# fancifulland2718/mujoco_InverseDynamicsTest

Measured on AMD Instinct MI355X. Metric: mj_inverse evals/sec, humanoid 27-DoF, batch=65536 @ 1/2/4/8 MI355X vs host CPU, higher is better.
Workload: dtype f64; 1 GPU; humanoid 27-DoF mj_inverse (skipstage NONE), contacts disabled, nefc=0, full mjData mirror written; per_gpu_batch=65536, global_batch=65536, parallelism=dp1

## Files before the change

include/mjhip.h:

```cpp
#ifndef MJHIP_H_
#define MJHIP_H_

#include <stddef.h>
#include <stdint.h>

#include "mjhip_fields.h"

#ifdef __cplusplus
extern "C" {
#endif

#if defined(_WIN32)
  #define MJHIP_API __declspec(dllexport)
#else
  #define MJHIP_API __attribute__((visibility("default")))
#endif

typedef double mjtNum;
typedef unsigned char mjtByte;

#define mjhipPI      3.14159265358979323846
#define mjhipMINVAL  1E-15
#define mjhipMAXVAL  1E+10
#define mjhipMINIMP  0.0001
// ... 197 lines not shown
MJHIP_API int mjhip_contextCreate(const mjhipModel* m, int device, int capacity,
                                  mjhipContext** out);
MJHIP_API int mjhip_contextCreateCapped(const mjhipModel* m, int device, int capacity,
                                        int max_contacts, int max_rows, mjhipContext** out);
MJHIP_API void mjhip_contextFree(mjhipContext* c);
MJHIP_API int mjhip_contextCapacity(const mjhipContext* c);
MJHIP_API const char* mjhip_contextFastKernel(const mjhipContext* c);
MJHIP_API int mjhip_contextFastKernelLds(const mjhipContext* c);
MJHIP_API int mjhip_contextLoadKernel(mjhipContext* c, const void* image, size_t size,
                                      const char* name, unsigned long long signature,
                                      int cmode);
MJHIP_API int mjhip_contextLastPath(const mjhipContext* c);
MJHIP_API int mjhip_contextConstStores(const mjhipContext* c);
MJHIP_API int mjhip_contextConstLaunches(const mjhipContext* c);
MJHIP_API int mjhip_contextQmHandoff(const mjhipContext* c);
MJHIP_API const char* mjhip_contextConstraintKernel(const mjhipContext* c);
MJHIP_API int mjhip_worklistCount(mjhipContext* c);
MJHIP_API void* mjhip_contextStream(mjhipContext* c);
MJHIP_API int mjhip_contextSetStream(mjhipContext* c, void* stream);

MJHIP_API int mjhip_inverseBatch(mjhipContext* c, int B,
                                 const mjtNum* qpos, const mjtNum* qvel, const mjtNum* qacc,
                                 mjtNum* qfrc_inverse, int skipstage, int skipsensor,
                                 int flags, int* status);

MJHIP_API int mjhip_forwardBatch(mjhipContext* c, int B, const mjtNum* qpos, const mjtNum* qvel,
                                 const mjtNum* ctrl, mjtNum* qacc, int flags, int* status);

MJHIP_API int mjhip_forwardBatchEx(mjhipContext* c, int B, const mjtNum* qpos,
                                   const mjtNum* qvel, const mjtNum* ctrl, const mjtNum* act,
// ... 134 lines not shown
```

mujoco_inversedynamicstest_amd/codegen.py:

```python
from __future__ import annotations

import hashlib
import re

import numpy as np

from . import fields

FREE, BALL, SLIDE, HINGE = 0, 1, 2, 3
STAGES = ("pos", "fac", "va")
FRAMES_IN_PASS1 = True
MAX_LDS_HINGES = 32
PREFETCH = 1
FUSE = True
VA_RECOMPUTE = False
QM_HANDOFF = True
QM_ORDER = "late"
QM_HANDOFF_MIN_B = 49152
VA_LDS_SLOTS = None
VA_KEEP_QFP = True
LDS_BUDGET = 40960
LANES = {"pos": 64, "fac": 64, "va": 64}
ALL_LANES = 64
ALL_WAVES = 1
NT_STORES = True
NT_TEMPORAL = None
NT_STAGES = ("pos", "fac", "va")
NT_SV_MIN_B = 49152
NT_LOAD_STAGES = ()
NT_LOAD_SV_STAGES = ("va",)
CONST_ONCE = True

# ... 186 lines not shown

def k_all_lds_bytes(m, va_slots=None) -> int:
  M = _Model(m, va_slots)
  return 8 * sum(_lds_doubles(m, M.va_nslot))


def qm_row(M, k) -> list:
  n, j = 0, k
  while j >= 0:
    n += 1
    j = M.dparent[j]
  return list(range(M.Madr[k], M.Madr[k] + n))


def qm_handoff_plan(m, va_slots=None, order=None) -> dict:
  order = QM_ORDER if order is None else order
  assert order in ("early", "late"), order
  M = m if isinstance(m, _Model) else _Model(m, va_slots, handoff=False)
  m = M.m
  if not QM_HANDOFF or not FUSE or ALL_LANES > 64:
    return {}
  nreg, nqo = _lds_doubles(m, M.va_nslot, 64)
  rows = nreg // 64
  events = []
  M.dfs(lambda b: events.append(("pre", b)), lambda b: events.append(("post", b)))
  when = {ev: t for t, ev in enumerate(events)}
  free_from = {s: -1 for s in range(2 * len(M.trig), rows)}
  if m.nv > 0:
    free_from.update({rows + k: -1 for k in range(nqo // 64)})
  if not (VA_RECOMPUTE and FUSE):
    for j, h in M.trig.items():
      t = when[("pre", int(m.jnt_bodyid[j]))]
      free_from[2 * h] = free_from[2 * h + 1] = t
  produced = [(when[("post", M.dbody[k])], k) for k in range(M.nv) if not M.simplenum[k]]
  produced.sort(reverse=order == "late")
  plan, taken = {}, set()
  for t, k in produced:
    entries = qm_row(M, k)
    free = sorted((s for s in free_from if free_from[s] < t and s not in taken),
                  key=lambda s: (free_from[s], s), reverse=order == "late")
    if len(free) < len(entries):
      continue
    for a, s in zip(entries, free):
      plan[a] = s
      taken.add(s)
  return plan


def _ho_ref(M, slot, st) -> str:
  rows = _lds_doubles(M.m, M.va_nslot, 64)[0] // 64
  li, ls = _ll(st)
  return f"trig, {slot}, {ls}, {li}" if slot < rows else f"qo_lds, {slot - rows}, {ls}, {li}"


class _Model:

  def __init__(self, m, va_slots=None, handoff=None):
    self.m = m
    self.nbody, self.nv, self.nq, self.njnt = m.nbody, m.nv, m.nq, m.njnt
    self.parent = [int(x) for x in m.body_parentid]
# ... 20 lines not shown
      ms[i] = ms[i] + self.mass[i]
      if i:
        ms[self.parent[i]] = ms[self.parent[i]] + ms[i]
    self.subtree_mass = ms
    hinges = [j for j in range(m.njnt) if int(m.jnt_type[j]) == HINGE]
    self.trig = {j: h for h, j in enumerate(hinges)} if 0 < len(hinges) <= MAX_LDS_HINGES else {}
    if va_slots is None:
      va_slots = VA_LDS_SLOTS
    if va_slots is None:
      va_slots = va_lds_capacity(m)
    if VA_RECOMPUTE and FUSE:
      va_slots = 0
    self.va_slot, depth = va_slot_plan(m, va_slots)
    self.va_nslot = min(va_slots, depth)
    self.spatial = set(spatial_tendons(m))
    self.handoff = qm_handoff_plan(self) if handoff is None or handoff else {}
    self.consts, self.const_decls = {}, []
    g = np.asarray(m.opt["gravity"], dtype=float)
    self.has_gravcomp = bool(m.ngravcomp and not (self.dsbl & (1 << 5)) and
                             not (self.dsbl & (1 << 6)) and np.sqrt(g @ g) != 0)
    self.has_fluid = (m.opt["density"] > 0 or m.opt["viscosity"] > 0) and \
        not self.dsbl & (1 << 5)
    self.ten_terms = []
    for t in range(m.ntendon):
      adr, num = int(m.tendon_adr[t]), int(m.tendon_num[t])
      if t in self.spatial:
        self.ten_terms.append(None)
        continue
      self.ten_terms.append([(float(m.wrap_prm[w]), int(m.jnt_qposadr[m.wrap_objid[w]]),
                              int(m.jnt_dofadr[m.wrap_objid[w]]))
                             for w in range(adr, adr + num)])
# ... 35 lines not shown
class _Stage:

  def __init__(self, M: _Model, store_fields=None):
    self.M = M
    self.E = _Emitter()
    self.store_fields = store_fields
    self.stored = set()

  def st(self, field, k, expr):
    self.stored.add(field)
    if field == "qM" and k in self.M.handoff:
      self.E(f"{{ const double v_ = {expr};")
      if self.store_fields is None or field in self.store_fields:
        self.E(f"P_qM[{k}*64] = v_;")
      self.E(f"mjh::handQM<HO>({_ho_ref(self.M, self.M.handoff[k], 'pos')}, v_); }}")
      return
    if self.store_fields is None or field in self.store_fields:
      self.E(f"P_{field}[{k}*64] = {expr};")

  def stv(self, field, k0, arr, n):
    for c in range(n):
      self.st(field, k0 + c, f"{arr}[{c}]")

  def st_const(self, field, k, expr, decl=None):
    if not self.M.const_ok(field):
      self.st(field, k, expr)
      return
    if self.store_fields is not None and field not in self.store_fields:
      return
    M = self.M
# ... 565 lines not shown
  E.close()


def _gen_fac(M: _Model, store_fields=None) -> str:
  G = _Stage(M, store_fields)
  E, m = G.E, M.m
  nv = M.nv
  G.prologue()
  G.pointers(["qM", "qLD", "qLDiagInv"])
  rownnz = [int(x) for x in m.C_rownnz]
  rowadr = [int(x) for x in m.C_rowadr]
  colind = [int(x) for x in m.C_colind]
  mapM2C = [int(x) for x in m.mapM2C]
  for a in range(m.nM):
    E(f"const double M_{a} = mjh::takeQM<HO>({_ho_ref(M, M.handoff[a], 'fac')}, P_qM + {a}*64);"
      if a in M.handoff else f"const double M_{a} = P_qM[{a}*64];")
  E(f"double {', '.join(f'L_{c} = M_{mapM2C[c]}' for c in range(m.nC))};")
  for k in range(nv - 1, -1, -1):
    ra = rowadr[k]
    dk = ra + rownnz[k] - 1
    E(f"const double diaginv_{k} = 1 / L_{dk};")
    G.st("qLDiagInv", k, f"diaginv_{k}")
    if not M.simplenum[k]:
      for a in range(dk - 1, ra - 1, -1):
        ii = colind[a]
        E.open()
        E(f"double tmp = L_{a} * diaginv_{k};")
        for t in range(rownnz[ii]):
          E(f"L_{rowadr[ii] + t} += L_{ra + t} * -tmp;")
        E(f"L_{a} = tmp;")
        E.close()
# ... 499 lines not shown
           "int* __restrict__ efc_count, double* __restrict__ qo_lds, "
           "double* __restrict__ trig",
           "qfrc_out, status, efc_count, qo_lds, trig"),
}
_HO_PARAM = {"pos": ", bool HO = false", "fac": ", bool HO = false", "va": ""}
_GEN = {"pos": lambda M, sf: _gen_pos(M, sf), "fac": lambda M, sf: _gen_fac(M, sf),
        "va": lambda M, sf: _gen_va(M, sf)}


def generate(m, name: str, store_fields=None, extern_c: bool = False, shared: bool = False,
             va_slots=None, handoff=None) -> str:
  why = fast_path_supported(m)
  if why:
    raise ValueError(f"model '{name}' cannot use the straight-line kernels: {why}")
  M = _Model(m, va_slots, handoff)
  ho = {st: "" if not _HO_PARAM[st] else ", true" if M.handoff else ", false" for st in STAGES}
  nreg64 = _lds_doubles(m, M.va_nslot, 64)[0]
  assert 8 * sum(_lds_doubles(m, M.va_nslot)) <= LDS_BUDGET, \
      f"k_all_{name}: {8 * sum(_lds_doubles(m, M.va_nslot))} B of LDS, three workgroups per CU"
  assert all(0 <= s < sum(_lds_doubles(m, M.va_nslot, 64)) // 64 for s in M.handoff.values())
  assert len(set(M.handoff.values())) == len(M.handoff)
  bodies = {st: _GEN[st](M, store_fields) for st in STAGES}
  if NT_STORES:
    import re
    reread = set(re.findall(r"= P_(\w+)\[", bodies["fac"])) | ({"qM"} if M.handoff else set())
    later = set(re.findall(r"= P_(\w+)\[", "\n".join(bodies.values()))) - reread
    if NT_TEMPORAL is not None:
      reread, later = set(NT_TEMPORAL), set()
    store = re.compile(r"^(\s*)P_(\w+)\[(\d+)\*64\] = (.+);$")

    def nt(line):
      mt = store.match(line)
      if mt and mt.group(2) == "qM" and int(mt.group(3)) in M.handoff and "qM" in reread:
        return f"{mt.group(1)}MJH_NT_STORE_IF(HO, P_qM[{mt.group(3)}*64], {mt.group(4)});"
      if not mt or mt.group(2) in reread:
        return line
      if mt.group(2) in later:
        return (f"{mt.group(1)}MJH_NT_STORE_IF(SV, P_{mt.group(2)}[{mt.group(3)}*64], "
                f"{mt.group(4)});")
      return f"{mt.group(1)}MJH_NT_STORE(P_{mt.group(2)}[{mt.group(3)}*64], {mt.group(4)});"
# ... 16 lines not shown
        C.E(line)
    for (f, k), expr in M.consts.items():
      C.E(f"P_{f}[{k}*64] = {expr};")
    C.E("(void)mr; (void)blk; (void)lane;")
    const_text = C.E.text()
  if M.cmode in ("none", "list") and store_fields is None:
    elided = fd_elided(list(bodies.values()) + [const_text])
    bodies = {st: _elide_stores(b, elided) for st, b in bodies.items()}
    const_text = _elide_stores(const_text, elided)
  out = [f"// GENERATED by mujoco_inversedynamicstest_amd/codegen.py -- do not edit.",
         f"// model '{name}' (nq={m.nq} nv={m.nv} nbody={m.nbody}), hash {model_hash(m)}"]
  exact = exact_fp(m)
  if exact:
    out.append("#if defined(__clang__)\n#pragma clang fp contract(off)\n#endif")
  for st in STAGES:
    params, args = _SIG[st]
    out.append(f"template <bool SV = true, bool FD = false{_HO_PARAM[st]}>\n"
               f"MJH_HD void fast_{st}_{name}(const Mirror& mr, int blk, int lane, int B, "
               f"{params}) {{\n{bodies[st]}\n}}\n")
  const_call = ""
  if CONST_ONCE:
    out.append(f"template <bool FD = false>\n"
               f"MJH_HD void fast_const_{name}(const Mirror& mr, int blk, int lane) {{\n"
               f"{const_text}\n}}\n")
    const_call = (f"  if (fd) fast_const_{name}<true>(mr, blk, lane);\n"
                  f"  else fast_const_{name}<false>(mr, blk, lane);\n")
  out.append(f"""MJH_HD void fast_body_{name}(
    const Mirror& mr, int blk, int lane, int B, const double* __restrict__ qpos_in,
    const double* __restrict__ qvel_in, const double* __restrict__ qacc_in,
    double* __restrict__ qfrc_out, int* __restrict__ status, int* __restrict__ worklist,
    int* __restrict__ worklist_count, int* __restrict__ worklist_next,
    int* __restrict__ efc_count) {{
  double trig[{nreg64}];   // LDS on the device (k_pos's trig, then k_va's cdof stack)
  double qo_lds[{64 * max(M.nv, 1)}];             // LDS on the device (k_va; the qM hand-off)
  const bool fd = mr.fd_elide && blk >= mr.full_blk;   // mjd_inverseFD's perturbed blocks
""" + const_call + "".join(f"  if (fd) fast_{st}_{name}<true, true{ho[st]}>(mr, blk, lane, B, {_SIG[st][1]});\n"
              f"  else fast_{st}_{name}<true, false{ho[st]}>(mr, blk, lane, B, {_SIG[st][1]});\n"
              for st in STAGES)
             + (f"""  if (qfrc_out && (long)blk*64 + lane < B) {{
    for (int k = 0; k < {M.nv}; k++) qfrc_out[((long)blk*64 + lane)*{M.nv} + k] = qo_lds[lane*{M.nv} + k];
  }}
""" if M.cmode != "all" else "  (void)qo_lds;\n") + "}\n")
  out.append("#if defined(__HIPCC__)")
  for st in STAGES:
    params, args = _SIG[st]
    tail = ""
    nl = LANES[st]
    sub = 64 // nl
    if st == "pos":
      params = params.replace(", double* __restrict__ trig", "")
      params = params.replace(", double* __restrict__ qo_lds", "")
      args = args.replace(", qo_lds", ", nullptr")
      decl = f"  __shared__ double trig[{max(1, 2 * len(M.trig) * nl)}];\n"
    elif st == "va":
      params = params.replace(", double* __restrict__ qo_lds", "")
      params = params.replace(", double* __restrict__ trig", "")
      decl = f"  __shared__ double qo_lds[{nl * max(M.nv, 1)}];\n"
      if M.va_slot:
        decl += f"  __shared__ double trig[{6 * M.va_nslot * nl}];\n"
      else:
        args = args.replace(", trig", ", nullptr")
      if M.cmode != "all":
        tail = (f"  if (!qfrc_out) return;\n  __syncthreads();\n"
                f"  const long r0 = (long)blockIdx.x*{nl};\n"
                f"  const long n = ((long)B - r0 < {nl} ? (long)B - r0 : {nl}) * {M.nv};\n"
                f"  double* dst = qfrc_out + r0*{M.nv};\n"
                f"  for (long r = threadIdx.x; r < n; r += {nl}) dst[r] = qo_lds[r];\n")
    else:
      params = params.replace(", const double* __restrict__ trig", "")
      params = params.replace(", const double* __restrict__ qo_lds", "")
      args = args.replace(", trig, qo_lds", ", nullptr, nullptr")
      decl = ""
    if sub == 1:
      bl = "blockIdx.x, threadIdx.x"
    else:
      bl = f"blockIdx.x / {sub}, (blockIdx.x % {sub})*{nl} + threadIdx.x"
    out.append(f"__global__ __launch_bounds__({nl}, 1) void k_{st}_{name}(Mirror mr, int B, "
               f"{params}) {{\n{decl}  fast_{st}_{name}(mr, {bl}, B, {args});\n"
               f"{tail}}}")
  nl = ALL_LANES
  if nl != 64:
    assert all(LANES[st] == nl for st in STAGES), "stage LDS indexing must match ALL_LANES"
  sub = 64 // nl
  ntrig, nqo = _lds_doubles(m, M.va_nslot, nl)
  stk_decl = f"  __shared__ double trig[{6 * M.va_nslot * 64}];\n" if M.va_slot else ""
  stk_arg = "trig" if M.va_slot else "nullptr"
# ... 2 lines not shown
    fuse_tail = (f"  if (!qfrc_out) return;\n  __syncthreads();\n"
                 f"  const long r0 = (long)blockIdx.x*{nl};\n"
                 f"  const long n = ((long)B - r0 < {nl} ? (long)B - r0 : {nl}) * {M.nv};\n"
                 f"  double* dst = qfrc_out + r0*{M.nv};\n"
                 f"  for (long r = threadIdx.x; r < n; r += {nl}) dst[r] = qo_lds[r];\n")
  bl = "blk0 + blockIdx.x, threadIdx.x" if sub == 1 else \
      f"blk0 + blockIdx.x / {sub}, (blockIdx.x % {sub})*{nl} + threadIdx.x"
  fuse_tail = fuse_tail.replace("(long)blockIdx.x*", f"((long)blk0*{sub} + blockIdx.x)*")
  linkage = 'extern "C" ' if extern_c else ""
  tmpl = "" if extern_c else "template <bool SV, bool FD, bool HO>\n"
  sv = "true" if extern_c else "SV"
  kho = ho if extern_c else {st: ", HO" if _HO_PARAM[st] else "" for st in STAGES}

  def stage_calls(fd, ind="  "):
    return "\n".join(f"{ind}fast_{st}_{name}<{sv}, {fd}{kho[st]}>(mr, {bl}, B, "
                     f"{_SIG[st][1].replace('worklist_next', 'nullptr')});\n"
                     f"{ind}asm volatile(\"\" ::: \"memory\"); MJH_SCHED_FENCE(); MJH_PHASE({20 + k});"
                     for k, st in enumerate(STAGES))
  blkexpr = "blk0 + (int)blockIdx.x" if sub == 1 else f"blk0 + (int)blockIdx.x / {sub}"
  all_calls = stage_calls("false") if extern_c else (
      f"  if (FD && mr.fd_elide && {blkexpr} >= mr.full_blk) {{\n{stage_calls('true', '    ')}\n"
      f"  }} else {{\n{stage_calls('false', '    ')}\n  }}")
  out.append(f"""{tmpl}{linkage}__global__ __launch_bounds__({nl}, {ALL_WAVES}) void k_all_{name}(Mirror mr, int B,
    const double* __restrict__ qpos_in, const double* __restrict__ qvel_in,
    const double* __restrict__ qacc_in, double* __restrict__ qfrc_out, int* __restrict__ status,
    int* __restrict__ worklist, int* __restrict__ worklist_count, int* __restrict__ worklist_next,
    int* __restrict__ efc_count, const int* __restrict__ range) {{
  __shared__ double trig[{ntrig}];
  __shared__ double qo_lds[{nqo}];
  if (worklist_next && blockIdx.x == 0 && threadIdx.x == 0) *worklist_next = 0;
  int blk0 = 0;
  if (range) {{ blk0 = range[0] >> 6; B = range[1]; }}
  MJH_PHASE0(19, 27);
""" + all_calls + "\n" + fuse_tail + "}")
  if M.cmode == "all" and not extern_c:
    import re
    ab = _gen_acc(M)
    if NT_STORES:
      ab = re.sub(r"^(\s*)P_(\w+)\[(\d+)\*64\] = (.+);$",
                  lambda mt: f"{mt.group(1)}MJH_NT_STORE(P_{mt.group(2)}[{mt.group(3)}*64], "
                             f"{mt.group(4)});", ab, flags=re.M)
    out.append(f"MJH_HD void fast_acc_{name}(const Mirror& mr, int blk, int lane, int B, "
               f"{_SIG['va'][0]}) {{\n{ab}\n}}\n")
    out.append(f"""__global__ __launch_bounds__(64, 1) void k_acc_{name}(Mirror mr, int B,
    double* __restrict__ qfrc_out, int* __restrict__ status, int* __restrict__ efc_count) {{
  fast_acc_{name}(mr, blockIdx.x, threadIdx.x, B, qfrc_out, status, efc_count, nullptr,
                  nullptr);
}}
{"" if shared else "static "}void launch_skip_{name}(hipStream_t s, const Mirror& mr, int B, int skipstage,
                              double* qfrc_out, int* status, int* efc_count) {{
  (void)qfrc_out;      // raw RNE only: k_skip_rows assembles and writes the output
  if (skipstage == 1) {{
    hipLaunchKernelGGL(k_va_{name}, dim3((B + 63) / 64), dim3(64), 0, s, mr, B, nullptr,
                       status, efc_count);
  }} else {{
    hipLaunchKernelGGL(k_acc_{name}, dim3((B + 63) / 64), dim3(64), 0, s, mr, B, nullptr,
                       status, efc_count);
  }}
# ... 6 lines not shown
    assert textual <= M.va_stored, \
        f"k_vaskip: va stores outside the record: {textual - M.va_stored}"
    own = set(M.va_stored)
    skip_body = re.sub(r"(double\* __restrict__ P_(\w+) = mr\.\w+ \+ \(\(long\))blk(\*\d+\)\*64 \+ )lane;",
                       lambda mt: mt.group(0) if mt.group(2) in own else
                       f"{mt.group(1)}sblk{mt.group(3)}slane;", vb)
    skip_body = skip_body.replace("const bool cflag = ec[0] != 0;",
                                  "const bool cflag = ecs[0] != 0;")
    skip_body = skip_body.replace("MJH_NT_STORE_IF(SV, ", "MJH_NT_STORE_IF(true, ")
    skip_body = skip_body.replace("if constexpr (!FD) {", "if constexpr (false) {")
    assert "FD" not in re.sub(r"\w*FD\w+|\w+FD\w*", "", skip_body), "k_vaskip: FD left"
    skip_body = skip_body.replace("MJH_NT_LOAD_IF(SV, ", "MJH_NT_LOAD_IF(false, ")
    skip_body = _perturb_loads(skip_body, {"qvel": "pv", "qacc": "pa"})
    out.append(f"MJH_HD void fast_vaskip_{name}(const Mirror& mr, int blk, int lane, int sblk, "
               f"int slane, int B, const int* __restrict__ ecs, int pa, int pv, double eps, "
               f"{_SIG['va'][0]}) {{\n{skip_body}\n}}\n")
  if M.cmode in ("none", "list") and not extern_c:
    import re
    ab = _gen_acc(M)
    if NT_STORES:
      ab = re.sub(r"^(\s*)P_(\w+)\[(\d+)\*64\] = (.+);$",
                  lambda mt: f"{mt.group(1)}MJH_NT_STORE(P_{mt.group(2)}[{mt.group(3)}*64], "
                             f"{mt.group(4)});", ab, flags=re.M)
    out.append(f"MJH_HD void fast_acc_{name}(const Mirror& mr, int blk, int lane, int B, "
               f"{_SIG['va'][0]}) {{\n{ab}\n}}\n")
  if M.cmode in ("none", "list") and not extern_c:
    flag = ("  if (ecs[0] != 0) needfull[0] = 1;\n" if M.cmode == "list" else "")
    out.append(f"""// layout 1 over [off, B): per = 2nv perturbations per centre, the first nv of qacc, the
// next nv of qvel (engine_derivative_fd.c:646-699 order)
__global__ __launch_bounds__(64, 1) void k_vaskip_{name}(Mirror mr, int B, int off,
    int per, int sstride, int* __restrict__ efc_count, int* __restrict__ needfull, double eps) {{
  __shared__ double qo_lds[{64 * max(M.nv, 1)}];
{stk_decl}  const long gi = (long)off + (long)blockIdx.x*64 + threadIdx.x;
  if (gi >= B) return;
  const long si = (gi - off) / per * sstride;
  const int j = (int)((gi - off) % per);
  const int* ecs = efc_count + (si >> 6)*4*64 + (si & 63);
{flag}  fast_vaskip_{name}(mr, (int)(gi >> 6), (int)(gi & 63), (int)(si >> 6), (int)(si & 63), B,
                    ecs, j < {M.nv} ? j : -1, j < {M.nv} ? -1 : j - {M.nv}, eps, nullptr,
                    nullptr, efc_count, qo_lds, {stk_arg});
# ... 30 lines not shown
    kbody = f"  fast_const_{name}(mr, blockIdx.x, threadIdx.x);" if CONST_ONCE else "  (void)mr;"
    out.append(f"{linkage}__global__ __launch_bounds__(64) void k_const_{name}(Mirror mr) {{\n"
               f"{kbody}\n}}")
    if extern_c:
      out.append(f'extern "C" __device__ __attribute__((used)) int k_const_count_{name} = '
                 f"{nconst};")
    else:
      out.append(f"""{"" if shared else "static "}void launch_const_{name}(hipStream_t s, const Mirror& mr, int nblk) {{
  hipLaunchKernelGGL(k_const_{name}, dim3(nblk), dim3(64), 0, s, mr);
}}
{"" if shared else "static "}int const_stores_{name}() {{ return {nconst}; }}""")
  assert len(M.consts) == nconst, "a constant store emitted after fast_const was written"
  if extern_c:
    out.append(f'extern "C" __device__ __attribute__((used)) int k_qm_handoff_{name} = '
               f"{len(M.handoff)};")
  else:
    out.append(f"{'' if shared else 'static '}int qm_handoff_{name}() "
               f"{{ return {len(M.handoff) if FUSE else 0}; }}")
  out.append(f"""{"" if shared else "static "}void launch_fast_{name}(dim3 g, dim3 b, hipStream_t s, const Mirror& mr,
    int B, const double* qpos_in, const double* qvel_in, const double* qacc_in, double* qfrc_out,
    int* status, int* worklist, int* worklist_count, int* worklist_next, int* efc_count,
    const int* range) {{""")
  if FUSE:
    gb = "g, b" if ALL_LANES == 64 else f"dim3(g.x*{64 // ALL_LANES}), dim3({ALL_LANES})"
    variants = ((f"B >= {NT_SV_MIN_B}", "<true, false>"), ("true", "<false, false>")) \
        if not extern_c else (("true", ""),)
    if not extern_c and M.cmode in ("none", "list"):
      variants = ((f"mr.fd_elide && B >= {NT_SV_MIN_B}", "<true, true>"),
                  ("mr.fd_elide", "<false, true>")) + variants
    if not extern_c:
      out.append(f"  const bool ho = mr.qm_handoff > 1 || (mr.qm_handoff == 1 && "
                 f"B >= {QM_HANDOFF_MIN_B});")
      variants = tuple(x for cond, v in variants for x in
                       ([(f"ho && ({cond})", v[:-1] + ", true>")] if M.handoff else []) +
                       [(cond, v[:-1] + ", false>")])
      if not M.handoff:
        out.append("  (void)ho;")
    for cond, v in variants:
      out.append(f"  if ({cond}) {{\n    hipLaunchKernelGGL((k_all_{name}{v}), {gb}, 0, s, mr, B, "
                 f"qpos_in, qvel_in, qacc_in, qfrc_out, status, worklist, worklist_count, "
                 f"worklist_next, efc_count, range);\n    return;\n  }}")
  else:
    out.append("  if (range) return;   // device-side ranges need k_all")
    for st in STAGES:
      args = _SIG["va"][1].replace(", trig", "").replace(", qo_lds", "") if st == "va" else \
          _SIG[st][1].replace(", trig, qo_lds", "")
      gb = "g, b" if LANES[st] == 64 else f"dim3(g.x*{64 // LANES[st]}), dim3({LANES[st]})"
      out.append(f"  hipLaunchKernelGGL(k_{st}_{name}, {gb}, 0, s, mr, B, {args});")
  out.append("}")
  if FUSE and not extern_c:
    out.append(f"{'' if shared else 'static '}int lds_fast_{name}() {{\n"
               f"  hipFuncAttributes a;\n  size_t n = 0;")
    for _, v in variants:
      out.append(f"  if (hipFuncGetAttributes(&a, (const void*)k_all_{name}{v}) != hipSuccess) "
                 f"return -1;\n  n = a.sharedSizeBytes > n ? a.sharedSizeBytes : n;")
    out.append("  return (int)n;\n}")
  else:
    out.append(f"{'' if shared else 'static '}int lds_fast_{name}() {{ return 0; }}")
  out.append("#endif")
  if exact:
    out.append("#if defined(__clang__)\n#pragma clang fp contract(fast)\n#endif")
# ... 54 lines not shown
    if exact_fp(m):
      exact.append(generate(m, name, shared=True))
      main.append(f"void launch_fast_{name}(dim3, dim3, hipStream_t, const Mirror&, int, "
                  "const double*, const double*, const double*, double*, int*, int*, int*, "
                  "int*, int*, const int*);")
      if vaskip:
        main.append(f"void launch_vaskip_{name}(hipStream_t, const Mirror&, int, int, int, int, "
                    "int*, int*, double);")
      main.append(f"void launch_skip_{name}(hipStream_t, const Mirror&, int, int, double*, "
                  "int*, int*);")
      main.append(f"int lds_fast_{name}();")
      if CONST_ONCE:
        main.append(f"void launch_const_{name}(hipStream_t, const Mirror&, int);")
        main.append(f"int const_stores_{name}();")
      main.append(f"int qm_handoff_{name}();")
    else:
      main.append(generate(m, name))
    vaskip_fn = f"launch_vaskip_{name}" if vaskip else "nullptr"
    const = f"launch_const_{name}, const_stores_{name}" if CONST_ONCE else "nullptr, nullptr"
    reg.append(f'  {{0x{fields.model_signature(m):016x}ull, launch_fast_{name}, "{name}", '
               f'{CONSTRAINT_MODES[constraint_mode(m)]}, {vaskip_fn}, launch_skip_{name}, '
               f'lds_fast_{name}, {const}, qm_handoff_{name}}},')
  main.append("static const FastKernelEntry g_fast_kernels[] = {")
  main.extend(reg)
  main.append("  {0ull, nullptr, nullptr, 0, nullptr, nullptr, nullptr, nullptr, nullptr, "
              "nullptr}};")
  return "\n".join(main) + "\n", "\n".join(exact) + "\n"
```

mujoco_inversedynamicstest_amd/csrc/fast_kernels.h:

```cpp
#ifndef MJHIP_FAST_KERNELS_H_
#define MJHIP_FAST_KERNELS_H_

#include <hip/hip_runtime.h>

#include "engine_device.h"

struct FastKernelEntry {
  unsigned long long sig;
  void (*launch)(dim3, dim3, hipStream_t, const Mirror&, int, const double*, const double*,
                 const double*, double*, int*, int*, int*, int*, int*,
                 const int* );
  const char* name;
  int cmode;
  void (*launch_vaskip)(hipStream_t, const Mirror&, int, int, int, int, int*, int*, double);
  void (*launch_skip)(hipStream_t, const Mirror&, int, int, double*, int*, int*);
  int (*lds_bytes)();
  void (*launch_const)(hipStream_t, const Mirror&, int);
  int (*const_stores)();
  int (*qm_handoff)();
};

constexpr int kFastLdsBudget = 40960;

const FastKernelEntry* mjhip_fastKernels();
int mjhip_genSetTimerBuf(unsigned long long* p);
int mjhip_genExactSetTimerBuf(unsigned long long* p);

#endif
```

mujoco_inversedynamicstest_amd/csrc/mjhip.hip:

```cpp
#include <hip/hip_runtime.h>

#include <stdarg.h>
#include <stdio.h>
#include <stdlib.h>
#include <string.h>

#include <algorithm>
#include <memory>
#include <mutex>
#include <string>
#include <unordered_map>
#include <unordered_set>
#include <utility>
#include <vector>

#include "engine_device.h"
#include "fast_kernels.h"
#include "kernels.h"
#include "pair_program.h"
#include "rollout.h"
#include "transition_call.h"
extern template __global__ void k_constraint_coop<8, true, false, false>(mjhipModel, Mirror, int, const int*, const int*, const CoopPair*, const mjh::ContactParam*, const unsigned long long*, int, double*, int*);
extern template __global__ void k_constraint_coop<32, true, false, false>(mjhipModel, Mirror, int, const int*, const int*, const CoopPair*, const mjh::ContactParam*, const unsigned long long*, int, double*, int*);
#include "post_pass.h"
// ... 406 lines not shown
  int* prog_ipair = nullptr;
  unsigned long long* masks = nullptr;
  int npair = 0;
  bool boxpair = false;
  int coop = 16;
  bool spatial = false;
  unsigned long long sig = 0;
  hipModule_t rt_module = nullptr;
  hipFunction_t rt_fn = nullptr;
  FastKernelEntry rt{};
  std::string rt_name;
  hipDeviceptr_t rt_tbuf = nullptr;
  hipFunction_t rt_const_fn = nullptr;
  int rt_nconst = 0;
  int rt_nhand = 0;
  bool const_stale = true;
  int const_launches = 0;
  unsigned long long* tbuf = nullptr;
  mjhipTimerStat timer[mjhipNTIMER]{};
  unsigned long long traw[MJH_TSLOTS]{};
  hipEvent_t tev0 = nullptr, tev1 = nullptr;
  double* rollout_scratch = nullptr;
  double* transition_y = nullptr;
  size_t transition_y_n = 0;
};

static bool mjhip_modelUsesActivation(const mjhipModel* m) {
  if (m->na > 0) return true;
  for (int i = 0; i < m->nu; i++) {
    if (m->actuator_gaintype[i] == mjhipGAIN_MUSCLE || m->actuator_biastype[i] == mjhipBIAS_MUSCLE) {
// ... 506 lines not shown
  c->rt_module = mod;
  c->rt_fn = fn;
  c->rt_const_fn = cfn;
  c->rt_nconst = nconst;
  c->const_stale = true;
  const std::string hname = std::string("k_qm_handoff_") + name;
  hipDeviceptr_t nhp = nullptr;
  size_t nhbytes = 0;
  c->rt_nhand = 0;
  if (hipModuleGetGlobal(&nhp, &nhbytes, mod, hname.c_str()) != hipSuccess ||
      nhbytes != sizeof(int) ||
      hipMemcpy(&c->rt_nhand, (const void*)nhp, sizeof(int), hipMemcpyDeviceToHost) != hipSuccess) {
    c->rt_nhand = 0;
    (void)hipGetLastError();
  }
  size_t tbytes = 0;
  if (hipModuleGetGlobal(&c->rt_tbuf, &tbytes, mod, "mjh_tbuf") != hipSuccess ||
      tbytes != sizeof(void*)) {
    c->rt_tbuf = nullptr;
    (void)hipGetLastError();
  }
  c->rt_name = name;
  c->rt = FastKernelEntry{signature, nullptr, c->rt_name.c_str(), cmode};
  c->fast = &c->rt;
  c->wl_parity = 0;
  return hipMemset(c->worklist, 0, 2 * sizeof(int)) == hipSuccess ? MJHIP_OK : MJHIP_ERR_HIP;
}

MJHIP_API int mjhip_ccdBatch(mjhipContext* c, int n, const int* g1, const int* g2,
                             const mjtNum* pos1, const mjtNum* mat1, const mjtNum* pos2,
// ... 86 lines not shown
  return (c && c->fast) ? c->fast_lds : 0;
}

MJHIP_API int mjhip_contextLastPath(const mjhipContext* c) { return c ? c->last_path : -1; }

MJHIP_API int mjhip_contextConstStores(const mjhipContext* c) {
  if (!c || !c->fast) return 0;
  if (c->fast == &c->rt) return c->rt_nconst;
  return c->fast->const_stores ? c->fast->const_stores() : 0;
}

MJHIP_API int mjhip_contextQmHandoff(const mjhipContext* c) {
  if (!c || !c->fast) return 0;
  if (c->fast == &c->rt) return c->rt_nhand;
  return (c->mirror.qm_handoff && c->fast->qm_handoff) ? c->fast->qm_handoff() : 0;
}

MJHIP_API int mjhip_contextConstLaunches(const mjhipContext* c) {
  return c ? c->const_launches : 0;
}

static int ensure_const(mjhipContext* c) {
  if (!c->const_stale || !c->fast) return MJHIP_OK;
  if (mjhip_contextConstStores(c) > 0) {
    const int nblk = c->capacity / 64;
    if (c->fast == &c->rt) {
      void* args[] = {&c->mirror};
      HIPCHECK(hipModuleLaunchKernel(c->rt_const_fn, nblk, 1, 1, 64, 1, 1, 0, c->stream, args,
                                     nullptr));
    } else {
// ... 1760 lines not shown
```

mujoco_inversedynamicstest_amd/engine.py:

```python
from __future__ import annotations

import ctypes
import os

import numpy as np

from . import fields, host

_HERE = os.path.dirname(os.path.abspath(__file__))
LIB_PATH = os.environ.get("MJHIP_LIB") or os.path.join(_HERE, "libmjhip.so")

mjSTAGE_NONE, mjSTAGE_POS, mjSTAGE_VEL = 0, 1, 2
FLAG_DEVICE_PTRS, FLAG_MIRROR_INPUT, FLAG_NO_MIRROR, FLAG_GENERIC = 1, 2, 4, 8
ERR = {0: "OK", -1: "NO_DEVICE", -2: "ARG", -3: "HIP", -4: "MODEL", -5: "CAPACITY",
       1: "INSTANCE"}
INST_BITS = {1: "BADQPOS", 2: "BADQVEL", 4: "BADQACC", 8: "INERTIA", 16: "CNSTRFULL",
             32: "UNSUPPORTED"}

_D = ctypes.POINTER(ctypes.c_double)
_I = ctypes.POINTER(ctypes.c_int)
_V = ctypes.c_void_p

SIGNATURES = {
    "mjhip_version": (ctypes.c_char_p, []),
# ... 5 lines not shown
    "mjhip_contextCreate": (ctypes.c_int, [_V, ctypes.c_int, ctypes.c_int,
                                           ctypes.POINTER(_V)]),
    "mjhip_contextCreateCapped": (ctypes.c_int, [_V, ctypes.c_int, ctypes.c_int, ctypes.c_int,
                                                 ctypes.c_int, ctypes.POINTER(_V)]),
    "mjhip_contextFree": (None, [_V]),
    "mjhip_contextCapacity": (ctypes.c_int, [_V]),
    "mjhip_contextFastKernel": (ctypes.c_char_p, [_V]),
    "mjhip_contextFastKernelLds": (ctypes.c_int, [_V]),
    "mjhip_contextLoadKernel": (ctypes.c_int, [_V, _V, ctypes.c_size_t, ctypes.c_char_p,
                                               ctypes.c_ulonglong, ctypes.c_int]),
    "mjhip_worklistCount": (ctypes.c_int, [_V]),
    "mjhip_contextLastPath": (ctypes.c_int, [_V]),
    "mjhip_contextConstStores": (ctypes.c_int, [_V]),
    "mjhip_contextConstLaunches": (ctypes.c_int, [_V]),
    "mjhip_contextQmHandoff": (ctypes.c_int, [_V]),
    "mjhip_contextConstraintKernel": (ctypes.c_char_p, [_V]),
    "mjhip_contextStream": (_V, [_V]),
    "mjhip_contextSetStream": (ctypes.c_int, [_V, _V]),
    "mjhip_inverseBatch": (ctypes.c_int, [_V, ctypes.c_int, _V, _V, _V, _V, ctypes.c_int,
                                          ctypes.c_int, ctypes.c_int, _I]),
    "mjhip_forwardBatch": (ctypes.c_int, [_V, ctypes.c_int, _V, _V, _V, _V, ctypes.c_int, _I]),
    "mjhip_forwardBatchEx": (ctypes.c_int, [_V, ctypes.c_int, _V, _V, _V, _V, _V, _V, _V,
                                            ctypes.c_int, _I]),
    "mjhip_actuationBatch": (ctypes.c_int, [_V, ctypes.c_int, _V, _V, _V, _V, _V, ctypes.c_int,
                                            _I]),
    "mjhip_rolloutBatch": (ctypes.c_int, [_V, ctypes.c_int, ctypes.c_int, _V, _V, ctypes.c_int,
                                          _V, _V]),
    "mjhip_transitionFDBatch": (ctypes.c_int, [_V, ctypes.c_int, _V, _V, ctypes.c_int, _V]),
    "mjhip_transitionFDSlots": (ctypes.c_long, [_V, ctypes.c_int, ctypes.c_int, ctypes.c_int,
                                                ctypes.c_int]),
# ... 201 lines not shown
  def constraint_kernel(self):
    n = lib().mjhip_contextConstraintKernel(self.ctx)
    return n.decode() if n else None

  @property
  def last_path(self):
    return lib().mjhip_contextLastPath(self.ctx)

  @property
  def const_stores(self):
    return lib().mjhip_contextConstStores(self.ctx)

  @property
  def qm_handoff(self):
    return lib().mjhip_contextQmHandoff(self.ctx)

  @property
  def const_launches(self):
    return lib().mjhip_contextConstLaunches(self.ctx)

  def worklist_count(self):
    return lib().mjhip_worklistCount(self.ctx)

  def inverse(self, qpos=None, qvel=None, qacc=None, out=None, skipstage=mjSTAGE_NONE,
              skipsensor=0, mirror_input=False, status=False, generic=False):
    L = lib()
    flags = FLAG_GENERIC if generic else 0
    if mirror_input:
      B = int(qpos)
      flags |= FLAG_MIRROR_INPUT
# ... 429 lines not shown
```

mujoco_inversedynamicstest_amd/specialize.py:

```python
from __future__ import annotations

import ctypes
import hashlib
import os
import subprocess
import sys
import tempfile

from . import codegen, fields

_HERE = os.path.dirname(os.path.abspath(__file__))
CSRC = os.path.join(_HERE, "csrc")
HIPCC = os.environ.get("HIPCC", "/opt/rocm/bin/hipcc")
FLAGS = ["--genco", "--offload-arch=gfx950", "-O3", "-std=c++17", "-Wno-unused-value",
         "-Wno-unused-result"]


def cache_dir() -> str:
  if os.environ.get("MJHIP_KERNEL_CACHE"):
    return os.environ["MJHIP_KERNEL_CACHE"]
  base = os.environ.get("XDG_CACHE_HOME") or os.path.join(os.path.expanduser("~"), ".cache")
  return os.path.join(base, "mjhip_kernels")


# ... 4 lines not shown
  global _compiler_id
  if _compiler_id is None:
    r = subprocess.run([HIPCC, "--version"], capture_output=True, text=True)
    if r.returncode != 0:
      raise SpecializeError(f"{HIPCC} --version failed: {r.stderr[-400:]}")
    _compiler_id = HIPCC + "\n" + r.stdout
  return _compiler_id


class SpecializeError(RuntimeError):
  pass


def source(m) -> tuple[str, str]:
  name = f"rt_{codegen.model_hash(m)}"
  body = codegen.generate(m, name, extern_c=True)
  exact = ('#define MJH_CONTRACT_OFF 1\n#pragma clang fp contract(off)\n'
           if codegen.exact_fp(m) else '')
  src = ('#include <hip/hip_runtime.h>\n#define MJH_TBUF_EXTERN 1\n' + exact +
         f'#include "{os.path.join(CSRC, "engine_device.h")}"\n' + body)
  return name, src


def code_object(m) -> tuple[bytes, str, int, int]:
  why = codegen.fast_path_supported(m)
  if why:
    raise SpecializeError(f"no straight-line kernel for this model: {why}")
  name, src = source(m)
  h = hashlib.sha256(src.encode())
  h.update(" ".join(FLAGS).encode())
  h.update(compiler_id().encode())
# ... 59 lines not shown
```

Before: 230.6 million evals/s.

## Forward mass-matrix entries from pos to fac stage through registers

Result: faster. 236.3 million evals/s (median of 6 runs) (+2.5%).

```diff
diff --git a/include/mjhip.h b/include/mjhip.h
--- a/include/mjhip.h
+++ b/include/mjhip.h
@@ -235,6 +235,7 @@
 MJHIP_API int mjhip_contextConstStores(const mjhipContext* c);
 MJHIP_API int mjhip_contextConstLaunches(const mjhipContext* c);
 MJHIP_API int mjhip_contextQmHandoff(const mjhipContext* c);
+MJHIP_API int mjhip_contextQmForward(const mjhipContext* c);
 MJHIP_API const char* mjhip_contextConstraintKernel(const mjhipContext* c);
 MJHIP_API int mjhip_worklistCount(mjhipContext* c);
 MJHIP_API void* mjhip_contextStream(mjhipContext* c);
diff --git a/mujoco_inversedynamicstest_amd/codegen.py b/mujoco_inversedynamicstest_amd/codegen.py
--- a/mujoco_inversedynamicstest_amd/codegen.py
+++ b/mujoco_inversedynamicstest_amd/codegen.py
@@ -16,6 +16,8 @@
 VA_RECOMPUTE = False
 QM_HANDOFF = True
 QM_ORDER = "late"
+QM_FORWARD = 128
+QM_LDS = True
 QM_HANDOFF_MIN_B = 49152
 VA_LDS_SLOTS = None
 VA_KEEP_QFP = True
@@ -232,17 +234,53 @@
 
 
 def qm_handoff_plan(m, va_slots=None, order=None) -> dict:
+  return _qm_plans(m, va_slots, order)[0]
+
+
+def qm_forward_plan(m, va_slots=None) -> dict:
+  return _qm_plans(m, va_slots, None)[1]
+
+
+def _qm_plans(m, va_slots=None, order=None) -> tuple:
   order = QM_ORDER if order is None else order
   assert order in ("early", "late"), order
   M = m if isinstance(m, _Model) else _Model(m, va_slots, handoff=False)
+  if not QM_HANDOFF or not FUSE or ALL_LANES > 64:
+    return {}, {}
+  if order == "early" or QM_FORWARD <= 0:
+    return _qm_lds_plan(M, order, ()), {}
+  last_first = [k for _, k in sorted(_qm_produced(M), reverse=True)]
+  best = None
+  for n in range(len(last_first) + 1):
+    suffix = last_first[:n]
+    lds = _qm_lds_plan(M, order, suffix)
+    fwd = [k for k in suffix if M.Madr[k] not in lds]
+    nfwd = sum(len(qm_row(M, k)) for k in fwd)
+    if nfwd <= QM_FORWARD and (best is None or len(lds) + nfwd > best[0]):
+      best = (len(lds) + nfwd, lds, fwd)
+  _, lds, fwd = best
+  entries = sorted(a for k in fwd for a in qm_row(M, k))
+  return lds, {a: i for i, a in enumerate(entries)}
+
+
+def _qm_events(M) -> dict:
+  events = []
+  M.dfs(lambda b: events.append(("pre", b)), lambda b: events.append(("post", b)))
+  return {ev: t for t, ev in enumerate(events)}
+
+
+def _qm_produced(M) -> list:
+  when = _qm_events(M)
+  return [(when[("post", M.dbody[k])], k) for k in range(M.nv) if not M.simplenum[k]]
+
+
+def _qm_lds_plan(M, order, suffix) -> dict:
   m = M.m
-  if not QM_HANDOFF or not FUSE or ALL_LANES > 64:
+  if not QM_LDS:
     return {}
   nreg, nqo = _lds_doubles(m, M.va_nslot, 64)
   rows = nreg // 64
-  events = []
-  M.dfs(lambda b: events.append(("pre", b)), lambda b: events.append(("post", b)))
-  when = {ev: t for t, ev in enumerate(events)}
+  when = _qm_events(M)
   free_from = {s: -1 for s in range(2 * len(M.trig), rows)}
   if m.nv > 0:
     free_from.update({rows + k: -1 for k in range(nqo // 64)})
@@ -250,18 +288,25 @@
     for j, h in M.trig.items():
       t = when[("pre", int(m.jnt_bodyid[j]))]
       free_from[2 * h] = free_from[2 * h + 1] = t
-  produced = [(when[("post", M.dbody[k])], k) for k in range(M.nv) if not M.simplenum[k]]
+  held = set(suffix)
+  produced = [x for x in _qm_produced(M) if x[1] not in held]
   produced.sort(reverse=order == "late")
   plan, taken = {}, set()
-  for t, k in produced:
+
+  def offer(t, k):
     entries = qm_row(M, k)
     free = sorted((s for s in free_from if free_from[s] < t and s not in taken),
                   key=lambda s: (free_from[s], s), reverse=order == "late")
     if len(free) < len(entries):
-      continue
+      return False
     for a, s in zip(entries, free):
       plan[a] = s
       taken.add(s)
+    return True
+  left_out = [offer(t, k) for t, k in produced].count(False)
+  if left_out:
+    for t, k in sorted(x for x in _qm_produced(M) if x[1] in held):
+      offer(t, k)
   return plan
 
 
@@ -312,7 +357,7 @@
     self.va_slot, depth = va_slot_plan(m, va_slots)
     self.va_nslot = min(va_slots, depth)
     self.spatial = set(spatial_tendons(m))
-    self.handoff = qm_handoff_plan(self) if handoff is None or handoff else {}
+    self.handoff, self.forward = _qm_plans(self) if handoff is None or handoff else ({}, {})
     self.consts, self.const_decls = {}, []
     g = np.asarray(m.opt["gravity"], dtype=float)
     self.has_gravcomp = bool(m.ngravcomp and not (self.dsbl & (1 << 5)) and
@@ -378,6 +423,12 @@
       if self.store_fields is None or field in self.store_fields:
         self.E(f"P_qM[{k}*64] = v_;")
       self.E(f"mjh::handQM<HO>({_ho_ref(self.M, self.M.handoff[k], 'pos')}, v_); }}")
+      return
+    if field == "qM" and k in self.M.forward:
+      self.E(f"{{ const double v_ = {expr};")
+      if self.store_fields is None or field in self.store_fields:
+        self.E(f"P_qM[{k}*64] = v_;")
+      self.E(f"if constexpr (HO) fw[{self.M.forward[k]}] = v_; }}")
       return
     if self.store_fields is None or field in self.store_fields:
       self.E(f"P_{field}[{k}*64] = {expr};")
@@ -973,7 +1024,8 @@
   mapM2C = [int(x) for x in m.mapM2C]
   for a in range(m.nM):
     E(f"const double M_{a} = mjh::takeQM<HO>({_ho_ref(M, M.handoff[a], 'fac')}, P_qM + {a}*64);"
-      if a in M.handoff else f"const double M_{a} = P_qM[{a}*64];")
+      if a in M.handoff else f"const double M_{a} = HO ? fw[{M.forward[a]}] : P_qM[{a}*64];"
+      if a in M.forward else f"const double M_{a} = P_qM[{a}*64];")
   E(f"double {', '.join(f'L_{c} = M_{mapM2C[c]}' for c in range(m.nC))};")
   for k in range(nv - 1, -1, -1):
     ra = rowadr[k]
@@ -1503,7 +1555,14 @@
   if why:
     raise ValueError(f"model '{name}' cannot use the straight-line kernels: {why}")
   M = _Model(m, va_slots, handoff)
-  ho = {st: "" if not _HO_PARAM[st] else ", true" if M.handoff else ", false" for st in STAGES}
+  sig = dict(_SIG)
+  nfw = len(M.forward)
+  if nfw:
+    sig["pos"] = (_SIG["pos"][0] + ", double* __restrict__ fw", _SIG["pos"][1] + ", fw")
+    sig["fac"] = (_SIG["fac"][0] + ", const double* __restrict__ fw", _SIG["fac"][1] + ", fw")
+  fw_decl = f"double fw[{nfw}];   // the forwarded qM entries (QM_FORWARD)\n" if nfw else ""
+  ho = {st: "" if not _HO_PARAM[st] else ", true" if M.handoff or M.forward else ", false"
+        for st in STAGES}
   nreg64 = _lds_doubles(m, M.va_nslot, 64)[0]
   assert 8 * sum(_lds_doubles(m, M.va_nslot)) <= LDS_BUDGET, \
       f"k_all_{name}: {8 * sum(_lds_doubles(m, M.va_nslot))} B of LDS, three workgroups per CU"
@@ -1512,7 +1571,8 @@
   bodies = {st: _GEN[st](M, store_fields) for st in STAGES}
   if NT_STORES:
     import re
-    reread = set(re.findall(r"= P_(\w+)\[", bodies["fac"])) | ({"qM"} if M.handoff else set())
+    reread = set(re.findall(r"= P_(\w+)\[", bodies["fac"])) | \
+        ({"qM"} if M.handoff or M.forward else set())
     later = set(re.findall(r"= P_(\w+)\[", "\n".join(bodies.values()))) - reread
     if NT_TEMPORAL is not None:
       reread, later = set(NT_TEMPORAL), set()
@@ -1559,7 +1619,7 @@
   if exact:
     out.append("#if defined(__clang__)\n#pragma clang fp contract(off)\n#endif")
   for st in STAGES:
-    params, args = _SIG[st]
+    params, args = sig[st]
     out.append(f"template <bool SV = true, bool FD = false{_HO_PARAM[st]}>\n"
                f"MJH_HD void fast_{st}_{name}(const Mirror& mr, int blk, int lane, int B, "
                f"{params}) {{\n{bodies[st]}\n}}\n")
@@ -1579,8 +1639,8 @@
   double trig[{nreg64}];   // LDS on the device (k_pos's trig, then k_va's cdof stack)
   double qo_lds[{64 * max(M.nv, 1)}];             // LDS on the device (k_va; the qM hand-off)
   const bool fd = mr.fd_elide && blk >= mr.full_blk;   // mjd_inverseFD's perturbed blocks
-""" + const_call + "".join(f"  if (fd) fast_{st}_{name}<true, true{ho[st]}>(mr, blk, lane, B, {_SIG[st][1]});\n"
-              f"  else fast_{st}_{name}<true, false{ho[st]}>(mr, blk, lane, B, {_SIG[st][1]});\n"
+""" + ("  " + fw_decl if nfw else "") + const_call + "".join(f"  if (fd) fast_{st}_{name}<true, true{ho[st]}>(mr, blk, lane, B, {sig[st][1]});\n"
+              f"  else fast_{st}_{name}<true, false{ho[st]}>(mr, blk, lane, B, {sig[st][1]});\n"
               for st in STAGES)
              + (f"""  if (qfrc_out && (long)blk*64 + lane < B) {{
     for (int k = 0; k < {M.nv}; k++) qfrc_out[((long)blk*64 + lane)*{M.nv} + k] = qo_lds[lane*{M.nv} + k];
@@ -1588,14 +1648,15 @@
 """ if M.cmode != "all" else "  (void)qo_lds;\n") + "}\n")
   out.append("#if defined(__HIPCC__)")
   for st in STAGES:
-    params, args = _SIG[st]
+    params, args = sig[st]
     tail = ""
     nl = LANES[st]
     sub = 64 // nl
     if st == "pos":
       params = params.replace(", double* __restrict__ trig", "")
       params = params.replace(", double* __restrict__ qo_lds", "")
-      args = args.replace(", qo_lds", ", nullptr")
+      params = params.replace(", double* __restrict__ fw", "")
+      args = args.replace(", qo_lds", ", nullptr").replace(", fw", ", nullptr")
       decl = f"  __shared__ double trig[{max(1, 2 * len(M.trig) * nl)}];\n"
     elif st == "va":
       params = params.replace(", double* __restrict__ qo_lds", "")
@@ -1614,7 +1675,8 @@
     else:
       params = params.replace(", const double* __restrict__ trig", "")
       params = params.replace(", const double* __restrict__ qo_lds", "")
-      args = args.replace(", trig, qo_lds", ", nullptr, nullptr")
+      params = params.replace(", const double* __restrict__ fw", "")
+      args = args.replace(", trig, qo_lds", ", nullptr, nullptr").replace(", fw", ", nullptr")
       decl = ""
     if sub == 1:
       bl = "blockIdx.x, threadIdx.x"
@@ -1647,7 +1709,7 @@
 
   def stage_calls(fd, ind="  "):
     return "\n".join(f"{ind}fast_{st}_{name}<{sv}, {fd}{kho[st]}>(mr, {bl}, B, "
-                     f"{_SIG[st][1].replace('worklist_next', 'nullptr')});\n"
+                     f"{sig[st][1].replace('worklist_next', 'nullptr')});\n"
                      f"{ind}asm volatile(\"\" ::: \"memory\"); MJH_SCHED_FENCE(); MJH_PHASE({20 + k});"
                      for k, st in enumerate(STAGES))
   blkexpr = "blk0 + (int)blockIdx.x" if sub == 1 else f"blk0 + (int)blockIdx.x / {sub}"
@@ -1665,7 +1727,7 @@
   int blk0 = 0;
   if (range) {{ blk0 = range[0] >> 6; B = range[1]; }}
   MJH_PHASE0(19, 27);
-""" + all_calls + "\n" + fuse_tail + "}")
+""" + ("  " + fw_decl if nfw else "") + all_calls + "\n" + fuse_tail + "}")
   if M.cmode == "all" and not extern_c:
     import re
     ab = _gen_acc(M)
@@ -1674,7 +1736,7 @@
                   lambda mt: f"{mt.group(1)}MJH_NT_STORE(P_{mt.group(2)}[{mt.group(3)}*64], "
                              f"{mt.group(4)});", ab, flags=re.M)
     out.append(f"MJH_HD void fast_acc_{name}(const Mirror& mr, int blk, int lane, int B, "
-               f"{_SIG['va'][0]}) {{\n{ab}\n}}\n")
+               f"{sig['va'][0]}) {{\n{ab}\n}}\n")
     out.append(f"""__global__ __launch_bounds__(64, 1) void k_acc_{name}(Mirror mr, int B,
     double* __restrict__ qfrc_out, int* __restrict__ status, int* __restrict__ efc_count) {{
   fast_acc_{name}(mr, blockIdx.x, threadIdx.x, B, qfrc_out, status, efc_count, nullptr,
@@ -1711,7 +1773,7 @@
     skip_body = _perturb_loads(skip_body, {"qvel": "pv", "qacc": "pa"})
     out.append(f"MJH_HD void fast_vaskip_{name}(const Mirror& mr, int blk, int lane, int sblk, "
                f"int slane, int B, const int* __restrict__ ecs, int pa, int pv, double eps, "
-               f"{_SIG['va'][0]}) {{\n{skip_body}\n}}\n")
+               f"{sig['va'][0]}) {{\n{skip_body}\n}}\n")
   if M.cmode in ("none", "list") and not extern_c:
     import re
     ab = _gen_acc(M)
@@ -1720,7 +1782,7 @@
                   lambda mt: f"{mt.group(1)}MJH_NT_STORE(P_{mt.group(2)}[{mt.group(3)}*64], "
                              f"{mt.group(4)});", ab, flags=re.M)
     out.append(f"MJH_HD void fast_acc_{name}(const Mirror& mr, int blk, int lane, int B, "
-               f"{_SIG['va'][0]}) {{\n{ab}\n}}\n")
+               f"{sig['va'][0]}) {{\n{ab}\n}}\n")
   if M.cmode in ("none", "list") and not extern_c:
     flag = ("  if (ecs[0] != 0) needfull[0] = 1;\n" if M.cmode == "list" else "")
     out.append(f"""// layout 1 over [off, B): per = 2nv perturbations per centre, the first nv of qacc, the
@@ -1781,9 +1843,12 @@
   if extern_c:
     out.append(f'extern "C" __device__ __attribute__((used)) int k_qm_handoff_{name} = '
                f"{len(M.handoff)};")
+    out.append(f'extern "C" __device__ __attribute__((used)) int k_qm_forward_{name} = {nfw};')
   else:
     out.append(f"{'' if shared else 'static '}int qm_handoff_{name}() "
                f"{{ return {len(M.handoff) if FUSE else 0}; }}")
+    out.append(f"{'' if shared else 'static '}int qm_forward_{name}() "
+               f"{{ return {nfw if FUSE else 0}; }}")
   out.append(f"""{"" if shared else "static "}void launch_fast_{name}(dim3 g, dim3 b, hipStream_t s, const Mirror& mr,
     int B, const double* qpos_in, const double* qvel_in, const double* qacc_in, double* qfrc_out,
     int* status, int* worklist, int* worklist_count, int* worklist_next, int* efc_count,
@@ -1799,9 +1864,9 @@
       out.append(f"  const bool ho = mr.qm_handoff > 1 || (mr.qm_handoff == 1 && "
                  f"B >= {QM_HANDOFF_MIN_B});")
       variants = tuple(x for cond, v in variants for x in
-                       ([(f"ho && ({cond})", v[:-1] + ", true>")] if M.handoff else []) +
+                       ([(f"ho && ({cond})", v[:-1] + ", true>")] if M.handoff or M.forward else []) +
                        [(cond, v[:-1] + ", false>")])
-      if not M.handoff:
+      if not (M.handoff or M.forward):
         out.append("  (void)ho;")
     for cond, v in variants:
       out.append(f"  if ({cond}) {{\n    hipLaunchKernelGGL((k_all_{name}{v}), {gb}, 0, s, mr, B, "
@@ -1810,8 +1875,8 @@
   else:
     out.append("  if (range) return;   // device-side ranges need k_all")
     for st in STAGES:
-      args = _SIG["va"][1].replace(", trig", "").replace(", qo_lds", "") if st == "va" else \
-          _SIG[st][1].replace(", trig, qo_lds", "")
+      args = sig["va"][1].replace(", trig", "").replace(", qo_lds", "") if st == "va" else \
+          sig[st][1].replace(", trig, qo_lds", "")
       gb = "g, b" if LANES[st] == 64 else f"dim3(g.x*{64 // LANES[st]}), dim3({LANES[st]})"
       out.append(f"  hipLaunchKernelGGL(k_{st}_{name}, {gb}, 0, s, mr, B, {args});")
   out.append("}")
@@ -1896,15 +1961,16 @@
         main.append(f"void launch_const_{name}(hipStream_t, const Mirror&, int);")
         main.append(f"int const_stores_{name}();")
       main.append(f"int qm_handoff_{name}();")
+      main.append(f"int qm_forward_{name}();")
     else:
       main.append(generate(m, name))
     vaskip_fn = f"launch_vaskip_{name}" if vaskip else "nullptr"
     const = f"launch_const_{name}, const_stores_{name}" if CONST_ONCE else "nullptr, nullptr"
     reg.append(f'  {{0x{fields.model_signature(m):016x}ull, launch_fast_{name}, "{name}", '
                f'{CONSTRAINT_MODES[constraint_mode(m)]}, {vaskip_fn}, launch_skip_{name}, '
-               f'lds_fast_{name}, {const}, qm_handoff_{name}}},')
+               f'lds_fast_{name}, {const}, qm_handoff_{name}, qm_forward_{name}}},')
   main.append("static const FastKernelEntry g_fast_kernels[] = {")
   main.extend(reg)
   main.append("  {0ull, nullptr, nullptr, 0, nullptr, nullptr, nullptr, nullptr, nullptr, "
-              "nullptr}};")
+              "nullptr, nullptr}};")
   return "\n".join(main) + "\n", "\n".join(exact) + "\n"
diff --git a/mujoco_inversedynamicstest_amd/csrc/fast_kernels.h b/mujoco_inversedynamicstest_amd/csrc/fast_kernels.h
--- a/mujoco_inversedynamicstest_amd/csrc/fast_kernels.h
+++ b/mujoco_inversedynamicstest_amd/csrc/fast_kernels.h
@@ -18,6 +18,7 @@
   void (*launch_const)(hipStream_t, const Mirror&, int);
   int (*const_stores)();
   int (*qm_handoff)();
+  int (*qm_forward)();
 };
 
 constexpr int kFastLdsBudget = 40960;
diff --git a/mujoco_inversedynamicstest_amd/csrc/mjhip.hip b/mujoco_inversedynamicstest_amd/csrc/mjhip.hip
--- a/mujoco_inversedynamicstest_amd/csrc/mjhip.hip
+++ b/mujoco_inversedynamicstest_amd/csrc/mjhip.hip
@@ -444,6 +444,7 @@
   hipFunction_t rt_const_fn = nullptr;
   int rt_nconst = 0;
   int rt_nhand = 0;
+  int rt_nfwd = 0;
   bool const_stale = true;
   int const_launches = 0;
   unsigned long long* tbuf = nullptr;
@@ -980,6 +981,14 @@
     c->rt_nhand = 0;
     (void)hipGetLastError();
   }
+  const std::string fname = std::string("k_qm_forward_") + name;
+  c->rt_nfwd = 0;
+  if (hipModuleGetGlobal(&nhp, &nhbytes, mod, fname.c_str()) != hipSuccess ||
+      nhbytes != sizeof(int) ||
+      hipMemcpy(&c->rt_nfwd, (const void*)nhp, sizeof(int), hipMemcpyDeviceToHost) != hipSuccess) {
+    c->rt_nfwd = 0;
+    (void)hipGetLastError();
+  }
   size_t tbytes = 0;
   if (hipModuleGetGlobal(&c->rt_tbuf, &tbytes, mod, "mjh_tbuf") != hipSuccess ||
       tbytes != sizeof(void*)) {
@@ -1096,6 +1105,12 @@
   if (!c || !c->fast) return 0;
   if (c->fast == &c->rt) return c->rt_nhand;
   return (c->mirror.qm_handoff && c->fast->qm_handoff) ? c->fast->qm_handoff() : 0;
+}
+
+MJHIP_API int mjhip_contextQmForward(const mjhipContext* c) {
+  if (!c || !c->fast) return 0;
+  if (c->fast == &c->rt) return c->rt_nfwd;
+  return (c->mirror.qm_handoff && c->fast->qm_forward) ? c->fast->qm_forward() : 0;
 }
 
 MJHIP_API int mjhip_contextConstLaunches(const mjhipContext* c) {
diff --git a/mujoco_inversedynamicstest_amd/engine.py b/mujoco_inversedynamicstest_amd/engine.py
--- a/mujoco_inversedynamicstest_amd/engine.py
+++ b/mujoco_inversedynamicstest_amd/engine.py
@@ -43,6 +43,7 @@
     "mjhip_contextConstStores": (ctypes.c_int, [_V]),
     "mjhip_contextConstLaunches": (ctypes.c_int, [_V]),
     "mjhip_contextQmHandoff": (ctypes.c_int, [_V]),
+    "mjhip_contextQmForward": (ctypes.c_int, [_V]),
     "mjhip_contextConstraintKernel": (ctypes.c_char_p, [_V]),
     "mjhip_contextStream": (_V, [_V]),
     "mjhip_contextSetStream": (ctypes.c_int, [_V, _V]),
@@ -274,6 +275,10 @@
   @property
   def qm_handoff(self):
     return lib().mjhip_contextQmHandoff(self.ctx)
+
+  @property
+  def qm_forward(self):
+    return lib().mjhip_contextQmForward(self.ctx)
 
   @property
   def const_launches(self):
diff --git a/mujoco_inversedynamicstest_amd/specialize.py b/mujoco_inversedynamicstest_amd/specialize.py
--- a/mujoco_inversedynamicstest_amd/specialize.py
+++ b/mujoco_inversedynamicstest_amd/specialize.py
@@ -42,7 +42,8 @@
 
 def source(m) -> tuple[str, str]:
   name = f"rt_{codegen.model_hash(m)}"
-  body = codegen.generate(m, name, extern_c=True)
+  handoff = None if os.environ.get("MJHIP_QM_HANDOFF", "1")[:1] != "0" else False
+  body = codegen.generate(m, name, extern_c=True, handoff=handoff)
   exact = ('#define MJH_CONTRACT_OFF 1\n#pragma clang fp contract(off)\n'
            if codegen.exact_fp(m) else '')
   src = ('#include <hip/hip_runtime.h>\n#define MJH_TBUF_EXTERN 1\n' + exact +
```
